# kessel/dune-pnp

Hardware: AMD Instinct MI355X
Metric: assembled DOFs/s + BiCGStab iters/s, 3-species PNP on pore.msh-refined (higher is better)
Workload: dtype f64; 1 GPU; config 3: stationary 3-ion PNP, test/pore_pnp/pore.msh refined k=4 x 1 mirrored copies; dofs=2214099, dofs_per_gpu=2214099, mesh_vertices=738033, triangles=1470464, parallelism=mesh partition (RCB) x1, preconditioner=ilu0, colors=4, sell_slots=5176768, blocks=5155025

## Files before the change

### dune-pnp_amd/csrc/assemble.hip

```cpp
#include <cstdlib>

#include <hip/hip_ext.h>

#include "element.h"
#include "kernels.h"

namespace pnp {

namespace {

template <int OP, int KC = 0>
__device__ __forceinline__ void store_block(double *__restrict__ vc, int lane, int s,
                                            const double *Kc) {
  constexpr int NK = OpTraits<OP>::NK;
  static_assert(!KC || OP == OP_PNP, "constant planes: the PNP operator only");
  constexpr int Q0 = KC ? 2 : 0;
#ifdef ASM_STORE_PLAIN
  store_vals<NK, Q0>(vc + size_t(s) * NK * kRows, lane, Kc);
#else
  store_vals_nt<NK, Q0>(vc + size_t(s) * NK * kRows, lane, Kc);
#endif
}

template <int NF>
__device__ __forceinline__ void residual_tail(const AsmArgs &a, int row, unsigned fl,
                                              const double (&R)[NF]) {
  double cv[NF];
#pragma unroll
  for (int f = 0; f < NF; f++) cv[f] = 0.0;
  if (fl & kRowFlagLoad) {
#pragma unroll
    for (int f = 0; f < NF; f++) cv[f] = a.cvec[size_t(row) * NF + f];
  }
#pragma unroll
  for (int f = 0; f < NF; f++) {
    const double rv = R[f] + cv[f];
    a.r[size_t(row) * NF + f] = ((fl >> f) & 1) ? 0.0 : rv;
  }
}

template <int OP, int JAC, int MINW, int FANR>
__global__ __launch_bounds__(256, MINW) void k_assemble(DevLayout L, AsmArgs a) {
  using T = OpTraits<OP>;
  constexpr int NF = T::NF, NK = T::NK;
  const int row = xcd_block(blockIdx.x, gridDim.x, L.xcd_remap) * blockDim.x + threadIdx.x;
  if (row >= L.n_owned) return;
  const int chunk = row / kRows, lane = row % kRows;
  const int off = L.chunk_off[chunk];
  const uint64_t meta = L.rowmeta[row];
  const int len = int(meta & 63);
  const bool closed = (meta >> 6) & 1;
  const unsigned brk = unsigned(meta >> 8);
  const int *__restrict__ cix = L.colidx + off + lane;
  double *__restrict__ vc = a.vals + size_t(off) * NK;

  const double2 pi2 = reinterpret_cast<const double2 *>(L.xy)[row];
  double ui[NF];
#pragma unroll
  for (int f = 0; f < NF; f++) ui[f] = a.x[size_t(row) * NF + f];
  double ai = 0, aq = 0;
  if constexpr (OP == OP_DIFF || OP == OP_DIFF_IE || OP == OP_POISSON) ai = a.aux0[row];
  if constexpr (OP == OP_POISSON) aq = a.aux1[row];
  if constexpr (OP == OP_PB) pb_fifth(ui[0], ai, aq);

  double R[NF], D[NK], P[NK], F[NK];
#pragma unroll
  for (int f = 0; f < NF; f++) R[f] = 0;
#pragma unroll
  for (int v = 0; v < NK; v++) D[v] = P[v] = F[v] = 0;

  auto next_slot = [&](int s) { return (s + 1 < len) ? s + 1 : (closed ? 1 : -1); };
  auto load_nb = [&](int j, double2 &p, double (&u)[NF], double &a0, double &a1) {
    p = reinterpret_cast<const double2 *>(L.xy)[j];
    load_nf<NF>(a.x, size_t(j), u);
    if constexpr (OP == OP_DIFF || OP == OP_DIFF_IE || OP == OP_POISSON) a0 = a.aux0[j];
    if constexpr (OP == OP_POISSON) a1 = a.aux1[j];
  };
  double2 pc, pn;
  double uc[NF], un[NF];
  double ac0 = 0, ac1 = 0, an0 = 0, an1 = 0;
  constexpr int NC = FANR > 0 ? FANR : 1;
  int cj[NC];
// ... 60 lines not shown
      for (int v = 0; v < NK; v++) P[v] = 0;
    }
    pc = pn;
#pragma unroll
    for (int f = 0; f < NF; f++) uc[f] = un[f];
    ac0 = an0;
    ac1 = an1;
    if (tn > 0) {
      pn = pp;
#pragma unroll
      for (int f = 0; f < NF; f++) un[f] = up[f];
      an0 = ap0;
      an1 = ap1;
    }
  }
  if constexpr (JAC) {
    if (closed) {
#pragma unroll
      for (int v = 0; v < NK; v++) F[v] += P[v];
      store_block<OP>(vc, lane, 1, F);
    }
    store_block<OP>(vc, lane, 0, D);
  }
  residual_tail<NF>(a, row, a.rowflag[row], R);
}

#ifndef ASM_SU
#define ASM_SU 4
#endif
template <int OP>
__host__ __device__ constexpr int asm_lds_rec() {
  return 2 + OpTraits<OP>::NF + (OP == OP_DIFF || OP == OP_DIFF_IE || OP == OP_POISSON) +
         (OP == OP_POISSON);
}
template <int OP>
constexpr int asm_kc() {
  return OP == OP_PNP;
}
constexpr int kPipeDw = 11;
template <class P>
__device__ __forceinline__ void lds_dma4(const P *src, uint32_t *dst_wave) {
  __builtin_amdgcn_global_load_lds(
      (const __attribute__((address_space(1))) void *)(src),
      (__attribute__((address_space(3))) void *)(dst_wave), 4, 0, 0);
}
__device__ __forceinline__ int const_ld(const int *p, int i) {
  return ((const __attribute__((address_space(4))) int *)(p))[i];
}
__device__ __forceinline__ int row_block_const(const DevLayout &L, int b, int nwg) {
  return L.blkmap ? const_ld(L.blkmap, xcd_block(b, nwg, 1)) : xcd_block(b, nwg, L.xcd_remap);
}
template <int OP, int JAC, int MINW, int FANR, int SPLIT = FANR, int STAGE = 0, int LDSG = 0,
          int KC = 0, int PIPE = 0>
__global__ __launch_bounds__(256, MINW) void k_assemble_ga(DevLayout L, AsmArgs a) {
  using T = OpTraits<OP>;
  constexpr int NF = T::NF, NK = T::NK, NS = FANR;
  constexpr bool AUX0 = OP == OP_DIFF || OP == OP_DIFF_IE || OP == OP_POISSON;
  constexpr bool AUX1 = OP == OP_POISSON;
  constexpr int RW = asm_lds_rec<OP>();
  static_assert(!PIPE || (JAC && FANR == 9 && !STAGE && !LDSG), "PIPE: the direct Jacobian walk");
  extern __shared__ double srec[];
  __shared__ uint32_t pfb[PIPE ? 4 * kPipeDw * kRows : 1];
  const int ntiles = (L.n_owned + 255) / 256, G = gridDim.x;
  const int wv = PIPE ? __builtin_amdgcn_readfirstlane(int(threadIdx.x) / kRows) : 0;
  const int ln = int(threadIdx.x) % kRows;
  uint32_t *const pw = pfb + (PIPE ? wv * kPipeDw * kRows : 0);
  int tile = blockIdx.x, b0 = -1, b1 = -1, b2 = -1, o0 = 0, o1 = 0, c1 = 0;
  auto tile_blk = [&](int t) { return t < ntiles ? row_block_const(L, t, ntiles) : -1; };
  auto wave_chunk = [&](int b) {
    return (b >= 0 && b * 256 + wv * kRows < L.n_owned) ? b * 4 + wv : -1;
  };
  auto prefetch = [&](int b, int off, int clen) {
    if (wave_chunk(b) < 0) return;
    const int r0 = b * 256 + wv * kRows;
    const int *cix = L.colidx + off + ln;
#pragma unroll
    for (int k = 1; k < NS; k++)
      lds_dma4(cix + (k < clen ? k : 0) * kRows, pw + (k - 1) * kRows);
    const uint32_t *m =
        reinterpret_cast<const uint32_t *>(L.rowmeta + min(r0 + ln, L.n_owned - 1));
    lds_dma4(m, pw + 8 * kRows);
    lds_dma4(m + 1, pw + 9 * kRows);
    lds_dma4(reinterpret_cast<const uint32_t *>(a.rowflag + r0) + (ln >> 2), pw + 10 * kRows);
  };
  if constexpr (PIPE) {
    if (tile >= ntiles) return;
    b0 = tile_blk(tile);
    b1 = tile_blk(tile + G);
    b2 = tile_blk(tile + 2 * G);
    int c0 = 0;
    if (wave_chunk(b0) >= 0) {
      o0 = const_ld(L.chunk_off, wave_chunk(b0));
      c0 = const_ld(L.chunk_len, wave_chunk(b0));
    }
    if (wave_chunk(b1) >= 0) {
      o1 = const_ld(L.chunk_off, wave_chunk(b1));
      c1 = const_ld(L.chunk_len, wave_chunk(b1));
    }
    prefetch(b0, o0, c0);
  }
  int o2 = 0, c2 = 0, b3 = -1;
  const auto advance = [&]() {
    tile += G;
    b0 = b1, o0 = o1;
    b1 = b2, o1 = o2, c1 = c2;
    b2 = b3;
    return b0 >= 0;
  };
  do {
    const int blk = PIPE ? b0 : row_block(L, blockIdx.x, gridDim.x);
    const int row0 = blk * blockDim.x + threadIdx.x;
    const bool live = row0 < L.n_owned;
    if (!PIPE && !LDSG && !live) return;
    const int row = live ? row0 : 0;
    const int chunk = row / kRows, lane = row % kRows;
    int cj[NS];
    uint64_t meta_pf = 0;
    unsigned fl_pf = 0;
    if constexpr (PIPE) {
      asm volatile("s_waitcnt vmcnt(0)" ::: "memory");
#pragma unroll
      for (int k = 1; k < NS; k++) cj[k] = int(pw[(k - 1) * kRows + ln]);
      meta_pf = uint64_t(pw[8 * kRows + ln]) | (uint64_t(pw[9 * kRows + ln]) << 32);
      fl_pf = (pw[10 * kRows + ln] >> (8 * (ln & 3))) & 0xffu;
      asm volatile("s_waitcnt lgkmcnt(0)" ::: "memory");
      prefetch(b1, o1, c1);
      o2 = c2 = 0;
      if (wave_chunk(b2) >= 0) {
        o2 = const_ld(L.chunk_off, wave_chunk(b2));
        c2 = const_ld(L.chunk_len, wave_chunk(b2));
      }
      b3 = tile_blk(tile + 3 * G);
      if (!live) continue;
    }
    const int off = PIPE ? o0 : L.chunk_off[chunk];
    const uint64_t meta = PIPE ? meta_pf : L.rowmeta[row];
    const int len = int(meta & 63);
    const bool closed = (meta >> 6) & 1;
    const unsigned brk = unsigned(meta >> 8);
    double *__restrict__ vc = a.vals + size_t(off) * NK;

    if constexpr (PIPE) {
    } else if constexpr (LDSG) {
      const uint16_t *__restrict__ lix = L.lidx + off + lane;
#pragma unroll
      for (int k = 1; k < NS; k++) {
        const int t = lix[(k < len ? k : 0) * kRows];
        cj[k] = k < len ? t : 0;
      }
    } else {
      const int *__restrict__ cix = L.colidx + off + lane;
#pragma unroll
      for (int k = 1; k < NS; k++) cj[k] = cix[(k < len ? k : 0) * kRows];
    }
    const double2 pi2 = reinterpret_cast<const double2 *>(L.xy)[row];
    double ui[NF];
    load_nf<NF>(a.x, size_t(row), ui);
    double ai = 0, aq = 0;
    if constexpr (AUX0) ai = a.aux0[row];
    if constexpr (AUX1) aq = a.aux1[row];
    if constexpr (OP == OP_PB) pb_fifth(ui[0], ai, aq);
    if constexpr (LDSG) {
      const int u0 = L.uptr[blk], cnt = L.uown[blk];
      constexpr int kSU = ASM_SU;
      int jj[kSU];
#pragma unroll
      for (int u = 0; u < kSU; u++) {
        const int k = int(threadIdx.x) + u * 256;
        jj[u] = k < cnt ? L.ulist[u0 + k] : -1;
      }
      double t[kSU][RW];
#pragma unroll
      for (int u = 0; u < kSU; u++)
        if (jj[u] >= 0) {
          const double2 p = reinterpret_cast<const double2 *>(L.xy)[jj[u]];
          t[u][0] = p.x;
          t[u][1] = p.y;
          double uu[NF];
          load_nf<NF>(a.x, size_t(jj[u]), uu);
#pragma unroll
// ... 100 lines not shown
#pragma unroll
              for (int v = 0; v < NK; v++) F[v] = P[v];
            } else {
              put(s, P);
            }
#pragma unroll
            for (int v = 0; v < NK; v++) P[v] = Ct[v];
          }
        } else if constexpr (JAC) {
          put(s, P);
#pragma unroll
          for (int v = 0; v < NK; v++) P[v] = 0;
        }
      }
    }
    if constexpr (JAC) {
      if (closed) {
#pragma unroll
        for (int v = 0; v < NK; v++) F[v] += P[v];
        store_block<OP, KC>(vc, lane, 1, F);
      }
      store_block<OP, KC>(vc, lane, 0, D);
    }
    residual_tail<NF>(a, row, PIPE ? fl_pf : unsigned(a.rowflag[row]), R);
  } while (PIPE && advance());
}

template <int OP>
__global__ __launch_bounds__(256) void k_mass_apply(DevLayout L, double tau, double pi, int cyl,
                                                    const double *__restrict__ xo,
                                                    double *__restrict__ cvec) {
  constexpr int NF = OpTraits<OP>::NF;
  const int row = blockIdx.x * blockDim.x + threadIdx.x;
  if (row >= L.n_owned) return;
  const int chunk = row / kRows, lane = row % kRows;
  const int off = L.chunk_off[chunk];
  const uint64_t meta = L.rowmeta[row];
  const int len = int(meta & 63);
  const bool closed = (meta >> 6) & 1;
  const int *cix = L.colidx + off + lane;
  const double2 pi2 = reinterpret_cast<const double2 *>(L.xy)[row];
  double acc = 0;
  for (int s = 1; s < len; ++s) {
    const int t = (s + 1 < len) ? s + 1 : (closed ? 1 : -1);
    if (t < 0 || ((meta >> (8 + s)) & 1)) continue;
    const int b = cix[s * kRows], c = cix[t * kRows];
    const double2 pb2 = reinterpret_cast<const double2 *>(L.xy)[b];
// ... 45 lines not shown
  double nx = ty / len, ny = -tx / len;
  if (nx * (po.x - pa.x) + ny * (po.y - pa.y) > 0) {
    nx = -nx;
    ny = -ny;
  }
  const double gp0 = factor * gf[0][0] * cp, gp1 = factor * gf[0][1] * cp;
  out[2 * size_t(k)] = (-factor * gf[1][0] + gp0) * nx + (-factor * gf[1][1] + gp1) * ny;
  const double r = cm / cp;
  out[2 * size_t(k) + 1] =
      (-factor * gf[2][0] - gp0 * r) * nx + (-factor * gf[2][1] - gp1 * r) * ny;
}

}

hipError_t launch_ion_flux(int ns, const int4 *seg, const double *xy, const double *x, int cyl,
                           double pi, double *out, hipStream_t s) {
  if (ns == 0) return hipSuccess;
  hipLaunchKernelGGL(k_ion_flux, dim3((ns + 255) / 256), dim3(256), 0, s, ns, seg, xy, x, cyl, pi,
                     out);
  return hipGetLastError();
}

constexpr bool kAsmPipeDefault = false;

template <int OP>
static int launch_pipe(const DevLayout &L, const AsmArgs &a, int cap, hipStream_t s, hipEvent_t t0,
                       hipEvent_t t1) {
  if constexpr (asm_kc<OP>()) {
    const auto kern = k_assemble_ga<OP, 1, 3, 9, 6, 0, 0, 1, 1>;
    static const int resident = [&] {
      int dev = 0, cus = 0, per_cu = 0;
      if (hipGetDevice(&dev) != hipSuccess ||
          hipDeviceGetAttribute(&cus, hipDeviceAttributeMultiprocessorCount, dev) != hipSuccess ||
          hipOccupancyMaxActiveBlocksPerMultiprocessor(&per_cu, kern, 256, 0) != hipSuccess)
        return 0;
      return per_cu * cus;
    }();
    const int ntiles = (L.n_owned + 255) / 256;
    int g = resident >= 8 ? resident / 8 * 8 : 8;
    if (g > ntiles) g = ntiles;
    if (cap > 0 && g > cap) g = cap;
    hipExtLaunchKernelGGL(kern, dim3(g), dim3(256), 0, s, t0, t1, 0, L, a);
    return 1;
  } else {
    return 0;
  }
// ... 18 lines not shown
  }();
  const int fanr = !fanr_ok ? 0 : (L.max_slots <= 9 ? 9 : (L.max_slots <= 12 ? 12 : 0));
  static const int lds_env = [] {
    const char *e = getenv("PNP_ASM_LDS");
    return e ? (atoi(e) == 1 ? 1 : 0) : -1;
  }();
  static const bool cold_hint = [] {
    const char *e = getenv("PNP_ASM_COLD_HINT");
    return !(e && e[0] == '0');
  }();
  const auto lds_walk = [&](int nk) {
    return lds_env == 1 ||
           (lds_env < 0 && (size_t(L.n_owned) * 7 * size_t(nk) * 8 > (size_t(512) << 20) ||
                            (cold_hint && a.cold)));
  };
  static const bool pipe_on = [] {
    const char *e = getenv("PNP_ASM_PIPE");
    return e ? atoi(e) != 0 : kAsmPipeDefault;
  }();
  static const int pipe_cap = [] {
    const char *e = getenv("PNP_ASM_PIPE_GRID");
    return (e && atoi(e) >= 1) ? atoi(e) : 0;
  }();
  int piped = 0;
#define PNP_ASM_CASE(OPK)                                                          \
  case OPK:                                                                        \
    if (!fanr && a.jac)                                                            \
      hipExtLaunchKernelGGL((k_assemble<OPK, 1, 3, 0>), grid, block, 0, s, t0, t1, 0, L, a);     \
    else if (!fanr)                                                                \
      hipExtLaunchKernelGGL((k_assemble<OPK, 0, 4, 0>), grid, block, 0, s, t0, t1, 0, L, a);     \
    else if (!a.jac && fanr == 9 && ga && lds_env == 1 && L.uown &&                 \
             size_t(L.unmax) * asm_lds_rec<OPK>() * 8 <= 53 * 1024)                    \
      hipExtLaunchKernelGGL((k_assemble_ga<OPK, 0, 3, 9, 9, 0, 1>), grid, block,         \
                         size_t(L.unmax) * asm_lds_rec<OPK>() * 8, s, t0, t1, 0, L, a);             \
    else if (!a.jac && fanr == 9 && ga)                                            \
      hipExtLaunchKernelGGL((k_assemble_ga<OPK, 0, 3, 9>), grid, block, 0, s, t0, t1, 0, L, a);  \
    else if (!a.jac)                                                               \
      hipExtLaunchKernelGGL((k_assemble<OPK, 0, 4, 12>), grid, block, 0, s, t0, t1, 0, L, a);    \
    else if (ga == 1 && fanr == 9)                                                 \
      hipExtLaunchKernelGGL((k_assemble_ga<OPK, 1, 3, 9>), grid, block, 0, s, t0, t1, 0, L, a);  \
    else if (ga == 2 && fanr == 9)                                                 \
      hipExtLaunchKernelGGL((k_assemble_ga<OPK, 1, 2, 9>), grid, block, 0, s, t0, t1, 0, L, a);  \
    else if (ga == 3 && fanr == 9)                                                 \
      hipExtLaunchKernelGGL((k_assemble_ga<OPK, 1, 3, 9, 5>), grid, block, 0, s, t0, t1, 0, L, a); \
    else if (ga == 4 && fanr == 9 && asm_kc<OPK>() && a.kconst &&                   \
             lds_walk(OpTraits<OPK>::NK) && L.uown &&                               \
             size_t(L.unmax) * asm_lds_rec<OPK>() * 8 <= 53 * 1024)                    \
      hipExtLaunchKernelGGL((k_assemble_ga<OPK, 1, 3, 9, 6, 0, 1, asm_kc<OPK>()>), grid,  \
                         block, size_t(L.unmax) * asm_lds_rec<OPK>() * 8, s, t0, t1, 0, L, a); \
    else if (ga == 4 && fanr == 9 && asm_kc<OPK>() && a.kconst && pipe_on)         \
      piped = launch_pipe<OPK>(L, a, pipe_cap, s, t0, t1);                         \
    else if (ga == 4 && fanr == 9 && asm_kc<OPK>() && a.kconst)                    \
      hipExtLaunchKernelGGL((k_assemble_ga<OPK, 1, 3, 9, 6, 0, 0, asm_kc<OPK>()>), grid,  \
                         block, 0, s, t0, t1, 0, L, a);                             \
    else if (ga == 4 && fanr == 9 && lds_walk(OpTraits<OPK>::NK) && L.uown &&       \
             size_t(L.unmax) * asm_lds_rec<OPK>() * 8 <= 53 * 1024)                    \
      hipExtLaunchKernelGGL((k_assemble_ga<OPK, 1, 3, 9, 6, 0, 1>), grid, block,         \
                         size_t(L.unmax) * asm_lds_rec<OPK>() * 8, s, t0, t1, 0, L, a);             \
    else if (ga == 4 && fanr == 9)                                                 \
      hipExtLaunchKernelGGL((k_assemble_ga<OPK, 1, 3, 9, 6>), grid, block, 0, s, t0, t1, 0, L, a); \
    else if (ga == 5 && fanr == 9)                                                 \
      hipExtLaunchKernelGGL((k_assemble_ga<OPK, 1, 3, 9, 3>), grid, block, 0, s, t0, t1, 0, L, a); \
    else if (ga == 6 && fanr == 9)                                                 \
      hipExtLaunchKernelGGL((k_assemble_ga<OPK, 1, 3, 9, 6, 1>), grid, block, 0, s, t0, t1, 0, L, a); \
    else if (fanr == 12)                                                           \
      hipExtLaunchKernelGGL((k_assemble<OPK, 1, 3, 12>), grid, block, 0, s, t0, t1, 0, L, a);    \
    else if (waves == 3)                                                           \
      hipExtLaunchKernelGGL((k_assemble<OPK, 1, 3, 9>), grid, block, 0, s, t0, t1, 0, L, a);     \
    else                                                                           \
      hipExtLaunchKernelGGL((k_assemble<OPK, 1, 4, 9>), grid, block, 0, s, t0, t1, 0, L, a);     \
    break;
  switch (a.kind) {
    PNP_ASM_CASE(OP_PNP)
    PNP_ASM_CASE(OP_PNP_IE)
    PNP_ASM_CASE(OP_PB)
    PNP_ASM_CASE(OP_DIFF)
    PNP_ASM_CASE(OP_DIFF_IE)
    PNP_ASM_CASE(OP_POISSON)
  default:
    return hipErrorInvalidValue;
  }
#undef PNP_ASM_CASE
  if (pipelined) *pipelined = piped;
  return hipGetLastError();
}

hipError_t launch_mass_apply(const DevLayout &L, int kind, double tau, double pi, int cylindrical,
                             const double *x_old, double *cvec, hipStream_t s) {
  if (L.n_owned == 0) return hipSuccess;
  dim3 grid((L.n_owned + 255) / 256), block(256);
  if (kind == OP_PNP_IE)
    hipLaunchKernelGGL(k_mass_apply<OP_PNP_IE>, grid, block, 0, s, L, tau, pi, cylindrical, x_old,
                       cvec);
  else if (kind == OP_DIFF_IE)
    hipLaunchKernelGGL(k_mass_apply<OP_DIFF_IE>, grid, block, 0, s, L, tau, pi, cylindrical,
                       x_old, cvec);
  else
    return hipErrorInvalidValue;
  return hipGetLastError();
}

}
```

### dune-pnp_amd/csrc/ctx.cc

```cpp
#include <hip/hip_runtime.h>
#include <rccl/rccl.h>
#include <rocsolver/rocsolver.h>

#include <algorithm>
#include <queue>
#include <random>
#include <chrono>
#include <condition_variable>
#include <map>
#include <unordered_map>
#include <mutex>
#include <cmath>
#include <cstdio>
#include <cstdlib>
#include <cstring>
#include <memory>
#include <string>
#include <vector>

#include "../../include/pnp_capi.h"
#include "amg.h"
#include "gmres_small.h"
#include "idr_small.h"
#include "kernels.h"
// ... 107 lines not shown
      d_usrc;
  DBuf<double> lvals, uvals, tsgs;
  int split_of = 0;
  int ilu_f32 = [] {
    const char *e = std::getenv("PNP_ILU_F32");
    const int v = e ? std::atoi(e) : 2;
    return (v >= 0 && v <= 3) ? v : 2;
  }();
  int ilu_eff() const { return (ilu_f32 >= 2 && nf == 1) ? 1 : ilu_f32; }
  int ilu_fac() const { return ilu_eff() == 3 ? 2 : ilu_eff(); }
  int f32_now() const { return split_of == 2 ? ilu_fac() : 0; }
  DBuf<float> ilu_y32buf;
  float *ilu_y32() const {
    return (split_of == 2 && ilu_eff() == 3 && !ilu_flow_opt) ? ilu_y32buf.p : nullptr;
  }
  int ilu_fused = 1;
  int amg_fallback = 0;
  int ilu_retry = 1;
  int twored_opt = [] {
    const char *ev = std::getenv("PNP_BICG_TWORED");
    return ev ? (std::atoi(ev) != 0 ? 1 : 0) : -1;
  }();
  DBuf<int> d_blkmap;
  DBuf<int> d_rowoff, d_rowcol;
  DBuf<int> d_blk_int, d_blk_bnd;
  int n_blk_int = 0, n_blk_bnd = 0;
  bool split_spmv = false;
  pnp::DevLayout sub_layout(bool interior) const {
    pnp::DevLayout d = dl;
    d.blkmap = interior ? d_blk_int.p : d_blk_bnd.p;
    const int n = interior ? n_blk_int : n_blk_bnd;
    d.blkcount = n > 0 ? n : -1;
    return d;
  }
  hipStream_t cstream = nullptr;
  hipEvent_t ev_ready = nullptr, ev_halo = nullptr;
  DBuf<double> scrub;
  bool fd_built = false, fd_mode = false;
  int fd_opt = 0;
  int fd_ne = 0;
  DBuf<int> fd_etri, fd_cdata;
  DBuf<long long> fd_rptr;
  DBuf<double> fd_jel;
  int csr_pat = -1, csr_nf = 0;
  long long csr_nnz = 0;
  DBuf<int> csr_rowptr, csr_col, csr_src;
// ... 3183 lines not shown
    if ((rc = up(c->d_rowoff, ro, "rowoff")) || (rc = up(c->d_rowcol, rcol, "rowcol"))) {
      g_err = c->err;
      return rc;
    }
  }
  {
    const char *e = getenv("PNP_BLKMAP");
    if (!(e && atoi(e) == 0) && L.n_owned > 0) {
      int nblk = (L.n_owned + 255) / 256;
      std::vector<double> key(nblk);
      for (int b = 0; b < nblk; b++) {
        int r = 256 * b, cc = L.rowcolor[r];
        double lo = L.color_ptr[cc], hi = L.color_ptr[cc + 1];
        key[b] = (r - lo) / std::max(1.0, hi - lo);
      }
      std::vector<int> order(nblk);
      for (int b = 0; b < nblk; b++) order[b] = b;
      std::stable_sort(order.begin(), order.end(), [&](int a, int b) { return key[a] < key[b]; });
      if ((rc = up(c->d_blkmap, order, "blkmap"))) {
        g_err = c->err;
        return rc;
      }
      c->dl.blkmap = c->d_blkmap.p;
    }
  }
  {
    const pnp::Mesh &mg = c->mesh;
    auto ekey = [](int a, int b) {
      if (a > b) std::swap(a, b);
      return (long long)a << 32 | (unsigned)b;
    };
    std::unordered_map<long long, int> opp;
    opp.reserve(size_t(mg.nb) * 2);
    for (int b = 0; b < mg.nb; b++) opp[ekey(mg.bseg[2 * b], mg.bseg[2 * b + 1])] = -1;
    for (int e = 0; e < mg.nt; e++)
      for (int k = 0; k < 3; k++) {
        auto it = opp.find(ekey(mg.tri[3 * e + k], mg.tri[3 * e + (k + 1) % 3]));
        if (it != opp.end() && it->second < 0) it->second = mg.tri[3 * e + (k + 2) % 3];
      }
    std::vector<int4> segs;
    for (int b = 0; b < mg.nb; b++) {
      const int a = mg.bseg[2 * b], cc = mg.bseg[2 * b + 1], lo = L.g2l[std::min(a, cc)];
      if (lo < 0 || lo >= L.n_owned) continue;
      const int o = opp[ekey(a, cc)];
      const int la = L.g2l[a], lc = L.g2l[cc], lop = o >= 0 ? L.g2l[o] : -1;
      if (la < 0 || lc < 0 || lop < 0) {
// ... 7 lines not shown
      g_err = c->err;
      return rc;
    }
  }
  c->dl.lchunk_len = c->d_lchunk_len.p;
  c->dl.lchunk_off = c->d_lchunk_off.p;
  c->dl.lcolidx = c->d_lcolidx.p;
  c->dl.uchunk_len = c->d_uchunk_len.p;
  c->dl.uchunk_off = c->d_uchunk_off.p;
  c->dl.ucolidx = c->d_ucolidx.p;
  if ((rc = up(c->d_chunk_len, L.chunk_len, "chunk_len")) ||
      (rc = up(c->d_chunk_off, L.chunk_off, "chunk_off")) ||
      (rc = up(c->d_colidx, L.colidx, "colidx")) || (rc = up(c->d_rowmeta, L.rowmeta, "rowmeta")) ||
      (rc = up(c->d_xy, xy, "xy")) || (rc = up(c->d_l2g, L.l2g, "l2g")) ||
      (rc = up(c->d_send_idx, L.send_idx, "send_idx")) ||
      (rc = up(c->d_color_idx, L.color_idx, "color_idx")) ||
      (rc = up(c->d_rowcolor, L.rowcolor, "rowcolor"))) {
    g_err = c->err;
    return rc;
  }
  {
    const char *e = getenv("PNP_XCD_REMAP");
    c->dl.xcd_remap = (e && atoi(e) == 1) ? 1 : 0;
  }
  c->dl.n_owned = L.n_owned;
  c->dl.n_local = nloc;
  c->dl.nchunks = L.nchunks;
  c->dl.max_slots = L.chunk_len.empty() ? 0 : *std::max_element(L.chunk_len.begin(), L.chunk_len.end());
  c->dl.ncolors = int(L.color_ptr.size()) - 1;
  c->dl.chunk_len = c->d_chunk_len.p;
  c->dl.chunk_off = c->d_chunk_off.p;
  c->dl.colidx = c->d_colidx.p;
  c->dl.rowmeta = c->d_rowmeta.p;
  if (const char *ev = getenv("PNP_SPMV_LDS"); !(ev && atoi(ev) == 0)) {
    const int nblk = (L.n_owned + 255) / 256;
    std::vector<int> uptr(nblk + 1, 0), ulist;
    std::vector<uint16_t> lidx(size_t(L.nslots), 0);
    std::vector<int> cols, uown(nblk, 0);
    int umax = 0, unmax = 0;
    bool fits = true;
    const bool own_last = [] {
      const char *e = getenv("PNP_LIST_OWN_LAST");
      return !(e && e[0] == '0');
    }();
    for (int b = 0; b < nblk && fits; b++) {
      cols.clear();
// ... 855 lines not shown
  if (!c) return PNP_E_ARG;
  if (replacements) *replacements = c->idr_replacements;
  return PNP_OK;
}

extern "C" int pnp_idr_shadow(pnp_ctx *c, int32_t j, double *p) {
  if (!c || !p) return PNP_E_ARG;
  if (!c->idr_P.p || c->idr_P_s != c->idr_s || c->idr_P_nf != c->nf)
    return c->fail(PNP_E_STATE, "no IDR solve yet with the current PNP_OPT_IDR_S and operator");
  if (j < 0 || j >= c->idr_s) return c->fail(PNP_E_ARG, "shadow column out of range");
  hipSetDevice(c->device);
  return c->download_ext(c->idr_P.p + size_t(j) * size_t(c->idr_ld(false)), c->nf, p);
}

extern "C" int pnp_asm_row_flags(pnp_ctx *c, uint8_t *flags) {
  if (!c || !flags) return PNP_E_ARG;
  if (c->kind < 0) return c->fail(PNP_E_STATE, "no operator set (pnp_set_operator)");
  if (c->degree > 1) return c->fail(PNP_E_STATE, "row flags: P1 contexts only");
  std::memset(flags, 0xff, size_t(c->mesh.nv));
  for (int i = 0; i < c->L.n_owned; i++) flags[c->L.l2g[i]] = c->hrowflag[i];
  return PNP_OK;
}

extern "C" int pnp_asm_info(pnp_ctx *c, int64_t *full, int64_t *reused, int64_t *pipelined) {
  if (!c) return PNP_E_ARG;
  if (full) *full = c->asm_full;
  if (reused) *reused = c->asm_reused;
  if (pipelined) *pipelined = c->asm_piped;
  return PNP_OK;
}

extern "C" int pnp_amg_configure(pnp_ctx *c, const pnp_amg_opts *o) {
  if (!c || !o) return PNP_E_ARG;
  if (o->smoother != PNP_PREC_SSOR && o->smoother != PNP_PREC_ILU0 &&
      o->smoother != PNP_PREC_JACOBI && o->smoother != PNP_PREC_SSOR_NATURAL)
    return c->fail(PNP_E_ARG, "AMG smoother must be SSOR, SSOR_NATURAL, ILU0 or JACOBI");
  if (o->coarse_target < 1 || o->coarse_target > pnp::kAmgMaxCoarse || o->max_levels < 2 ||
      o->max_levels > pnp::kAmgMaxLevels || !(o->omega > 0 && o->omega <= 2) ||
      o->coarse_sweeps < 1 || o->coarse_sweeps > 8 || o->level0_presmooth < -1 ||
      o->level0_presmooth > 1)
    return c->fail(PNP_E_ARG, "AMG options out of range");
  const bool rebuild = o->coarse_target != c->amg_opts.coarse_target ||
                       o->max_levels != c->amg_opts.max_levels;
  c->amg_opts = *o;
  if (rebuild) c->amg_built = false;
  c->amg_valid = false;
// ... 685 lines not shown
```

### dune-pnp_amd/csrc/kernels.h

```cpp
#pragma once

#include <hip/hip_runtime.h>

#include <cstdint>

namespace pnp {

constexpr int kRows = 64;

__device__ __forceinline__ int xcd_block(int b, int nwg, int on = 1) {
  if (!on) return b;
  const int q = nwg / 8, r = nwg % 8, xcd = b % 8;
  return (xcd < r ? xcd * (q + 1) : r * (q + 1) + (xcd - r) * q) + b / 8;
}

typedef double double2_a8 __attribute__((ext_vector_type(2), aligned(8)));
template <int NF>
__device__ __forceinline__ void load_nf(const double *__restrict__ x, size_t j, double (&o)[NF]) {
  const double *b = x + size_t(NF) * j;
  int f = 0;
#pragma unroll
  for (; f + 1 < NF; f += 2) {
    const double2_a8 a = *reinterpret_cast<const double2_a8 *>(b + f);
    o[f] = a.x;
    o[f + 1] = a.y;
  }
  if (f < NF) o[f] = b[f];
}
template <int NF>
__device__ __forceinline__ void store_nf(double *__restrict__ x, size_t j, const double (&v)[NF]) {
  double *b = x + size_t(NF) * j;
  int f = 0;
#pragma unroll
// ... 130 lines not shown
template <int NF, int PAT>
__host__ __device__ __forceinline__ void mask_rows(double *B, unsigned dm, bool diag) {
#pragma unroll
  for (int f = 0; f < NF; f++)
#pragma unroll
    for (int g = 0; g < NF; g++) {
      const int v = pat_index(PAT, f, g);
      if (v >= 0 && ((dm >> f) & 1)) B[v] = (diag && f == g) ? 1.0 : 0.0;
    }
}

struct DevLayout {
  int n_owned = 0, n_local = 0, nchunks = 0, ncolors = 0;
  int max_slots = 0;
  int xcd_remap = 0;
  const int *chunk_len = nullptr;
  const int *chunk_off = nullptr;
  const int *colidx = nullptr;
  const uint64_t *rowmeta = nullptr;
  const double *xy = nullptr;
  const int *color_idx = nullptr;
  const uint8_t *rowcolor = nullptr;
  const int *blkmap = nullptr;
  int blkcount = 0;
  const int *lchunk_len = nullptr, *lchunk_off = nullptr, *lcolidx = nullptr;
  const int *uchunk_len = nullptr, *uchunk_off = nullptr, *ucolidx = nullptr;
  const uint8_t *dmask = nullptr;
  const int *uptr = nullptr, *ulist = nullptr;
  const uint16_t *lidx = nullptr;
  int umax = 0;
  const int *uown = nullptr;
  int unmax = 0;
  const int *lsx_ptr = nullptr, *lsx_list = nullptr, *usx_ptr = nullptr, *usx_list = nullptr;
  const uint8_t *lperm = nullptr, *uperm = nullptr, *lpinv = nullptr, *upinv = nullptr;
  const uint8_t *llen = nullptr, *ulen = nullptr, *ldl = nullptr;
  const uint16_t *lsx_idx = nullptr, *usx_idx = nullptr;
  int sx_max = 0;
};

template <int NF>
__device__ __forceinline__ unsigned row_mask(const DevLayout &L, int row) {
  unsigned dm = 0;
#pragma unroll
  for (int f = 0; f < NF; f++) dm |= unsigned(L.dmask[size_t(row) * NF + f] != 0) << f;
  return dm;
}

constexpr unsigned kRowFlagMask = 7, kRowFlagLoad = 8;

struct AsmArgs {
  int kind;
  int jac;
  double l_b, c0, tau, pi, dt, z;
  int cylindrical;
  const double *x;
  const double *aux0;
  const double *aux1;
  const double *cvec;
  const uint8_t *dmask;
  const uint8_t *rowflag;
  double *r;
// ... 234 lines not shown
```

### dune-pnp_amd/python/pnp_amd/__init__.py

```python
from __future__ import annotations

import ctypes as C
import os
from dataclasses import dataclass

import numpy as np

HERE = os.path.dirname(os.path.abspath(__file__))
PKG_ROOT = os.path.dirname(os.path.dirname(HERE))
REPO_ROOT = os.path.dirname(PKG_ROOT)
LIB_PATH = os.environ.get("PNP_AMD_LIB") or os.path.join(PKG_ROOT, "libpnp_amd.so")
HEADER = os.path.join(REPO_ROOT, "include", "pnp_capi.h")

OK, E_ARG, E_HIP, E_RCCL, E_BREAKDOWN, E_NOT_CONVERGED, E_IO, E_MESH, E_STATE = \
    0, -1, -2, -3, -4, -5, -6, -7, -8
OP_PNP, OP_PNP_IMPLICIT_EULER, OP_PB, OP_DIFF, OP_DIFF_IMPLICIT_EULER, OP_POISSON = range(6)
PREC_NONE, PREC_SSOR, PREC_ILU0, PREC_JACOBI, PREC_AMG, PREC_SSOR_NATURAL = range(6)
METHOD_BICGSTAB, METHOD_CG, METHOD_GMRES, METHOD_FGMRES, METHOD_IDR = 0, 1, 2, 3, 4
(OPT_ILU_F32, OPT_ILU_FUSED_FACTOR, OPT_JAC_FD, OPT_BICG_TWORED, OPT_AMG_FALLBACK,
 OPT_GRAPH, OPT_SEQ_ORDER, OPT_ILU_FLOW, OPT_NAT_FLOW, OPT_ILU_RETRY,
 OPT_GMRES_RESTART, OPT_MATRIX_FREE, OPT_ASM_REUSE_CONST, OPT_IDR_S) = (1, 2, 3, 4, 5, 6, 7, 8,
                                                                        9, 10, 11, 12, 13, 14)
ASM_PIPE_ENV, ASM_PIPE_GRID_ENV = "PNP_ASM_PIPE", "PNP_ASM_PIPE_GRID"
ROW_FLAG_LOAD = 8
DEVICE_PTRS, JAC_FD = 1, 2
CREATE_ABSORB_THIN_COLOR = 1
PREC_BY_NAME = {"none": PREC_NONE, "nonprec": PREC_NONE, "ssor": PREC_SSOR, "ilu0": PREC_ILU0,
                "jacobi": PREC_JACOBI, "amg": PREC_AMG, "ssor_natural": PREC_SSOR_NATURAL}
MAX_SURFACES = 64


class PnpError(RuntimeError):
    def __init__(self, code, msg):
        super().__init__(f"pnp error {code}: {msg}")
        self.code = code


class _Mesh(C.Structure):
    _fields_ = [("nv", C.c_int32), ("coords", C.c_void_p), ("nt", C.c_int32),
                ("tri", C.c_void_p), ("nbseg", C.c_int32), ("bseg", C.c_void_p),
                ("bseg_group", C.c_void_p)]


class _Surface(C.Structure):
    _fields_ = [("coulomb_btype", C.c_int32), ("coulomb_flux", C.c_double),
                ("coulomb_potential", C.c_double), ("plus_btype", C.c_int32),
                ("plus_flux", C.c_double), ("plus_concentration", C.c_double),
# ... 700 lines not shown
    def asm_row_flags(self):
        out = np.zeros(self.mesh.nv, dtype=np.uint8)
        self._ck(lib().pnp_asm_row_flags(self.h, out.ctypes.data_as(C.c_void_p)))
        return out

    def probe_slot_stores(self, tile_elems=256, reps=20):
        o = _StoreProbe()
        self._ck(lib().pnp_probe_slot_stores(self.h, int(tile_elems), int(reps), C.byref(o)))
        return {k: getattr(o, k) for k, _ in _StoreProbe._fields_}

    def cache_scrub(self, nbytes=1 << 30):
        self._ck(lib().pnp_cache_scrub(self.h, C.c_int64(int(nbytes))))

    def timers(self, enable=None, reset=False):
        if enable is not None:
            self._ck(lib().pnp_timers_enable(self.h, int(bool(enable))))
        if reset:
            self._ck(lib().pnp_timers_reset(self.h))
        t = _Timers()
        self._ck(lib().pnp_timers_get(self.h, C.byref(t)))
        return {k: getattr(t, k) for k, _ in _Timers._fields_}


def header_symbols():
    import re
    txt = open(HEADER).read()
    return sorted(set(re.findall(r"^\s*(?:int|void|const char \*)\s*(pnp_\w+)\s*\(", txt, re.M)))


def header_constants():
    import re
    txt = open(HEADER).read()
    return {k: int(v) for k, v in re.findall(r"^\s*(PNP_\w+)\s*=\s*(-?\d+)\s*,?\s*$", txt, re.M)}
```

### include/pnp_capi.h

```cpp
#ifndef PNP_CAPI_H
#define PNP_CAPI_H

#include <stdint.h>

#ifdef __cplusplus
extern "C" {
#endif

#define PNP_CAPI_VERSION 1

enum {
  PNP_OK = 0,
  PNP_E_ARG = -1,
  PNP_E_HIP = -2,
  PNP_E_RCCL = -3,
  PNP_E_BREAKDOWN = -4,
  PNP_E_NOT_CONVERGED = -5,
  PNP_E_IO = -6,
  PNP_E_MESH = -7,
  PNP_E_STATE = -8
};

typedef struct pnp_ctx pnp_ctx;

// ... 181 lines not shown
  double omega;
} pnp_amg_stats;
int pnp_amg_info(pnp_ctx *ctx, pnp_amg_stats *stats);
int pnp_amg_aggregates(pnp_ctx *ctx, int32_t level, int32_t *agg);

enum {
  PNP_OPT_ILU_F32 = 1,
  PNP_OPT_ILU_FUSED_FACTOR = 2,
  PNP_OPT_JAC_FD = 3,
  PNP_OPT_BICG_TWORED = 4,
  PNP_OPT_AMG_FALLBACK = 5,
  PNP_OPT_GRAPH = 6,
  PNP_OPT_SEQ_ORDER = 7,
  PNP_OPT_ILU_FLOW = 8,
  PNP_OPT_NAT_FLOW = 9,
  PNP_OPT_ILU_RETRY = 10,
  PNP_OPT_GMRES_RESTART = 11,
  PNP_OPT_MATRIX_FREE = 12,
  PNP_OPT_ASM_REUSE_CONST = 13,
  PNP_OPT_IDR_S = 14
};
int pnp_set_option(pnp_ctx *ctx, int32_t option, int64_t value);
int pnp_asm_info(pnp_ctx *ctx, int64_t *full, int64_t *reused, int64_t *pipelined);
#define PNP_ROW_FLAG_LOAD 8
int pnp_asm_row_flags(pnp_ctx *ctx, uint8_t *flags);
int pnp_matfree_info(pnp_ctx *ctx, int64_t *applies, int64_t *value_assemblies);
int pnp_idr_info(pnp_ctx *ctx, int64_t *replacements);
int pnp_idr_shadow(pnp_ctx *ctx, int32_t j, double *p);

enum {
  PNP_CREATE_ABSORB_THIN_COLOR = 1
};
int pnp_set_create_option(int32_t option, int64_t value);
int pnp_get_create_option(int32_t option, int64_t *value);
int pnp_get_option(pnp_ctx *ctx, int32_t option, int64_t *value);

int pnp_linear_solve(pnp_ctx *ctx, const double *rhs, double *z, const pnp_solve_opts *opts,
                     pnp_solve_result *res);
int pnp_linear_solve_ex(pnp_ctx *ctx, const double *rhs, double *z, const pnp_solve_opts *opts,
                        pnp_solve_result *res, int32_t flags);

int pnp_solve_history(pnp_ctx *ctx, double *defects, int32_t cap, int32_t *n);

typedef struct {
  double reduction, abs_limit, min_linear_reduction;
  int32_t maxit, line_search_maxit;
// ... 80 lines not shown
```

Measured before the change: 55.29 billion assembled DOFs/s.

## Launch direct assembly walks as one-wave workgroups driven by a precomputed unit table

Builds a host-side table of per-wave assembly units holding the chunk index, offset and length, ordered by XCD and block map, and uploads it to the device. The non-pipelined direct assembly kernels now read this table through scalar constant loads instead of computing the block index and loading chunk_off per wave. They are launched by default as 64-thread workgroups, one wave per unit, in place of 256-thread blocks. The rowflag load is also moved earlier, next to the other row loads, to hide its latency. This trades an extra table and a different scheduling granularity for fewer dependent address loads at kernel start and finer wave dispatch.

Result: no change. 55.77 billion assembled DOFs/s, median of 6 (+0.9%).

```diff
diff --git a/dune-pnp_amd/csrc/assemble.hip b/dune-pnp_amd/csrc/assemble.hip
--- a/dune-pnp_amd/csrc/assemble.hip
+++ b/dune-pnp_amd/csrc/assemble.hip
@@ -37,6 +37,21 @@
     const double rv = R[f] + cv[f];
     a.r[size_t(row) * NF + f] = ((fl >> f) & 1) ? 0.0 : rv;
   }
+}
+
+__device__ __forceinline__ unsigned head_flag(const AsmArgs &a, int row) {
+#ifdef ASM_FLAG_TAIL
+  return 0;
+#else
+  return a.rowflag[row];
+#endif
+}
+__device__ __forceinline__ unsigned tail_flag(const AsmArgs &a, int row, unsigned fl) {
+#ifdef ASM_FLAG_TAIL
+  return a.rowflag[row];
+#else
+  return fl;
+#endif
 }
 
 template <int OP, int JAC, int MINW, int FANR>
@@ -58,6 +73,7 @@
   double ui[NF];
 #pragma unroll
   for (int f = 0; f < NF; f++) ui[f] = a.x[size_t(row) * NF + f];
+  const unsigned fl = head_flag(a, row);
   double ai = 0, aq = 0;
   if constexpr (OP == OP_DIFF || OP == OP_DIFF_IE || OP == OP_POISSON) ai = a.aux0[row];
   if constexpr (OP == OP_POISSON) aq = a.aux1[row];
@@ -164,7 +180,7 @@
     }
     store_block<OP>(vc, lane, 0, D);
   }
-  residual_tail<NF>(a, row, a.rowflag[row], R);
+  residual_tail<NF>(a, row, tail_flag(a, row, fl), R);
 }
 
 #ifndef ASM_SU
@@ -189,22 +205,37 @@
 __device__ __forceinline__ int const_ld(const int *p, int i) {
   return ((const __attribute__((address_space(4))) int *)(p))[i];
 }
+__device__ __forceinline__ int4 unit_ld(const int4 *p, int i) {
+  typedef int i4v __attribute__((ext_vector_type(4)));
+  const i4v e = ((const __attribute__((address_space(4))) i4v *)(p))[i];
+  return make_int4(e.x, e.y, e.z, e.w);
+}
+#ifdef ASM_HEAD_CHAIN
+constexpr bool kAsmUnits = false;
+#else
+constexpr bool kAsmUnits = true;
+#endif
 __device__ __forceinline__ int row_block_const(const DevLayout &L, int b, int nwg) {
   return L.blkmap ? const_ld(L.blkmap, xcd_block(b, nwg, 1)) : xcd_block(b, nwg, L.xcd_remap);
 }
 template <int OP, int JAC, int MINW, int FANR, int SPLIT = FANR, int STAGE = 0, int LDSG = 0,
-          int KC = 0, int PIPE = 0>
-__global__ __launch_bounds__(256, MINW) void k_assemble_ga(DevLayout L, AsmArgs a) {
+          int KC = 0, int PIPE = 0, int WG = 256>
+__global__ __launch_bounds__(WG, MINW) void k_assemble_ga(DevLayout L, AsmArgs a) {
   using T = OpTraits<OP>;
   constexpr int NF = T::NF, NK = T::NK, NS = FANR;
   constexpr bool AUX0 = OP == OP_DIFF || OP == OP_DIFF_IE || OP == OP_POISSON;
   constexpr bool AUX1 = OP == OP_POISSON;
   constexpr int RW = asm_lds_rec<OP>();
   static_assert(!PIPE || (JAC && FANR == 9 && !STAGE && !LDSG), "PIPE: the direct Jacobian walk");
+  static_assert(WG == 256 || (WG == kRows && kAsmUnits && !PIPE && !STAGE && !LDSG),
+                "one-wave workgroups: the walks without LDS, by the unit table");
+  constexpr bool UNITS = kAsmUnits && !PIPE;
   extern __shared__ double srec[];
   __shared__ uint32_t pfb[PIPE ? 4 * kPipeDw * kRows : 1];
   const int ntiles = (L.n_owned + 255) / 256, G = gridDim.x;
-  const int wv = PIPE ? __builtin_amdgcn_readfirstlane(int(threadIdx.x) / kRows) : 0;
+  const int wv = (PIPE || (UNITS && WG == 256))
+                     ? __builtin_amdgcn_readfirstlane(int(threadIdx.x) / kRows)
+                     : 0;
   const int ln = int(threadIdx.x) % kRows;
   uint32_t *const pw = pfb + (PIPE ? wv * kPipeDw * kRows : 0);
   int tile = blockIdx.x, b0 = -1, b1 = -1, b2 = -1, o0 = 0, o1 = 0, c1 = 0;
@@ -250,9 +281,24 @@
     return b0 >= 0;
   };
   do {
-    const int blk = PIPE ? b0 : row_block(L, blockIdx.x, gridDim.x);
-    const int row0 = blk * blockDim.x + threadIdx.x;
-    const bool live = row0 < L.n_owned;
+    int blk = 0, row0 = 0, off_u = 0, clen_u = 0;
+    bool live;
+    if constexpr (UNITS) {
+#ifndef ASM_KARG_LATE
+      asm volatile("" ::"s"(L.n_owned), "s"(L.colidx), "s"(L.rowmeta), "s"(L.xy), "s"(a.x),
+                   "s"(a.rowflag));
+#endif
+      const int b = blockIdx.x, u0 = (4 * (b / 8)) * 8 + b % 8;
+      const int4 e = unit_ld(L.units, WG == kRows ? b : u0 + 8 * wv);
+      if constexpr (LDSG) blk = unit_ld(L.units, u0).x / 4;
+      off_u = e.y, clen_u = e.z;
+      row0 = e.x * kRows + ln;
+      live = e.x >= 0 && row0 < L.n_owned;
+    } else {
+      blk = PIPE ? b0 : row_block(L, blockIdx.x, gridDim.x);
+      row0 = blk * blockDim.x + threadIdx.x;
+      live = row0 < L.n_owned;
+    }
     if (!PIPE && !LDSG && !live) return;
     const int row = live ? row0 : 0;
     const int chunk = row / kRows, lane = row % kRows;
@@ -275,7 +321,7 @@
       b3 = tile_blk(tile + 3 * G);
       if (!live) continue;
     }
-    const int off = PIPE ? o0 : L.chunk_off[chunk];
+    const int off = PIPE ? o0 : (UNITS ? off_u : L.chunk_off[chunk]);
     const uint64_t meta = PIPE ? meta_pf : L.rowmeta[row];
     const int len = int(meta & 63);
     const bool closed = (meta >> 6) & 1;
@@ -287,17 +333,18 @@
       const uint16_t *__restrict__ lix = L.lidx + off + lane;
 #pragma unroll
       for (int k = 1; k < NS; k++) {
-        const int t = lix[(k < len ? k : 0) * kRows];
+        const int t = lix[(k < (UNITS ? clen_u : len) ? k : 0) * kRows];
         cj[k] = k < len ? t : 0;
       }
     } else {
       const int *__restrict__ cix = L.colidx + off + lane;
 #pragma unroll
-      for (int k = 1; k < NS; k++) cj[k] = cix[(k < len ? k : 0) * kRows];
+      for (int k = 1; k < NS; k++) cj[k] = cix[(k < (UNITS ? clen_u : len) ? k : 0) * kRows];
     }
     const double2 pi2 = reinterpret_cast<const double2 *>(L.xy)[row];
     double ui[NF];
     load_nf<NF>(a.x, size_t(row), ui);
+    const unsigned fl_hd = PIPE ? 0u : head_flag(a, row);
     double ai = 0, aq = 0;
     if constexpr (AUX0) ai = a.aux0[row];
     if constexpr (AUX1) aq = a.aux1[row];
@@ -444,7 +491,7 @@
       }
       store_block<OP, KC>(vc, lane, 0, D);
     }
-    residual_tail<NF>(a, row, PIPE ? fl_pf : unsigned(a.rowflag[row]), R);
+    residual_tail<NF>(a, row, PIPE ? fl_pf : tail_flag(a, row, fl_hd), R);
   } while (PIPE && advance());
 }
 
@@ -536,6 +583,8 @@
 }
 
 constexpr bool kAsmPipeDefault = false;
+constexpr int kAsmWgDefault = kRows;
+constexpr int kAsmWg1 = kAsmUnits ? kRows : 256;
 
 template <int OP>
 static int launch_pipe(const DevLayout &L, const AsmArgs &a, int cap, hipStream_t s, hipEvent_t t0,
@@ -600,7 +649,26 @@
     const char *e = getenv("PNP_ASM_PIPE_GRID");
     return (e && atoi(e) >= 1) ? atoi(e) : 0;
   }();
+  static const int wg = [] {
+    const char *e = getenv("PNP_ASM_WG");
+    const int v = e ? atoi(e) : 0;
+    return (v == 64 || v == 256) && kAsmUnits ? v : (kAsmUnits ? kAsmWgDefault : 256);
+  }();
+  if (kAsmUnits && !L.units) return hipErrorInvalidValue;
+  const dim3 grid1(unsigned(asm_unit_count(L.n_owned))), block1(kRows);
   int piped = 0;
+#define PNP_ASM_DIRECT(OPK, JAC, SPLIT, KC)                                                     \
+  do {                                                                                          \
+    if constexpr (kAsmUnits) {                                                                  \
+      if (wg == kRows) {                                                                        \
+        hipExtLaunchKernelGGL((k_assemble_ga<OPK, JAC, 3, 9, SPLIT, 0, 0, KC, 0, kAsmWg1>),     \
+                              grid1, block1, 0, s, t0, t1, 0, L, a);                            \
+        break;                                                                                  \
+      }                                                                                         \
+    }                                                                                           \
+    hipExtLaunchKernelGGL((k_assemble_ga<OPK, JAC, 3, 9, SPLIT, 0, 0, KC>), grid, block, 0, s,  \
+                          t0, t1, 0, L, a);                                                     \
+  } while (0)
 #define PNP_ASM_CASE(OPK)                                                          \
   case OPK:                                                                        \
     if (!fanr && a.jac)                                                            \
@@ -612,7 +680,7 @@
       hipExtLaunchKernelGGL((k_assemble_ga<OPK, 0, 3, 9, 9, 0, 1>), grid, block,         \
                          size_t(L.unmax) * asm_lds_rec<OPK>() * 8, s, t0, t1, 0, L, a);             \
     else if (!a.jac && fanr == 9 && ga)                                            \
-      hipExtLaunchKernelGGL((k_assemble_ga<OPK, 0, 3, 9>), grid, block, 0, s, t0, t1, 0, L, a);  \
+      PNP_ASM_DIRECT(OPK, 0, 9, 0);                                                \
     else if (!a.jac)                                                               \
       hipExtLaunchKernelGGL((k_assemble<OPK, 0, 4, 12>), grid, block, 0, s, t0, t1, 0, L, a);    \
     else if (ga == 1 && fanr == 9)                                                 \
@@ -629,14 +697,13 @@
     else if (ga == 4 && fanr == 9 && asm_kc<OPK>() && a.kconst && pipe_on)         \
       piped = launch_pipe<OPK>(L, a, pipe_cap, s, t0, t1);                         \
     else if (ga == 4 && fanr == 9 && asm_kc<OPK>() && a.kconst)                    \
-      hipExtLaunchKernelGGL((k_assemble_ga<OPK, 1, 3, 9, 6, 0, 0, asm_kc<OPK>()>), grid,  \
-                         block, 0, s, t0, t1, 0, L, a);                             \
+      PNP_ASM_DIRECT(OPK, 1, 6, asm_kc<OPK>());                                    \
     else if (ga == 4 && fanr == 9 && lds_walk(OpTraits<OPK>::NK) && L.uown &&       \
              size_t(L.unmax) * asm_lds_rec<OPK>() * 8 <= 53 * 1024)                    \
       hipExtLaunchKernelGGL((k_assemble_ga<OPK, 1, 3, 9, 6, 0, 1>), grid, block,         \
                          size_t(L.unmax) * asm_lds_rec<OPK>() * 8, s, t0, t1, 0, L, a);             \
     else if (ga == 4 && fanr == 9)                                                 \
-      hipExtLaunchKernelGGL((k_assemble_ga<OPK, 1, 3, 9, 6>), grid, block, 0, s, t0, t1, 0, L, a); \
+      PNP_ASM_DIRECT(OPK, 1, 6, 0);                                                \
     else if (ga == 5 && fanr == 9)                                                 \
       hipExtLaunchKernelGGL((k_assemble_ga<OPK, 1, 3, 9, 3>), grid, block, 0, s, t0, t1, 0, L, a); \
     else if (ga == 6 && fanr == 9)                                                 \
@@ -659,6 +726,7 @@
     return hipErrorInvalidValue;
   }
 #undef PNP_ASM_CASE
+#undef PNP_ASM_DIRECT
   if (pipelined) *pipelined = piped;
   return hipGetLastError();
 }
diff --git a/dune-pnp_amd/csrc/ctx.cc b/dune-pnp_amd/csrc/ctx.cc
--- a/dune-pnp_amd/csrc/ctx.cc
+++ b/dune-pnp_amd/csrc/ctx.cc
@@ -153,6 +153,8 @@
     return ev ? (std::atoi(ev) != 0 ? 1 : 0) : -1;
   }();
   DBuf<int> d_blkmap;
+  std::vector<int> h_blkmap;
+  DBuf<int> d_units;
   DBuf<int> d_rowoff, d_rowcol;
   DBuf<int> d_blk_int, d_blk_bnd;
   int n_blk_int = 0, n_blk_bnd = 0;
@@ -3382,6 +3384,7 @@
         return rc;
       }
       c->dl.blkmap = c->d_blkmap.p;
+      c->h_blkmap = order;
     }
   }
   {
@@ -3435,6 +3438,17 @@
   {
     const char *e = getenv("PNP_XCD_REMAP");
     c->dl.xcd_remap = (e && atoi(e) == 1) ? 1 : 0;
+  }
+  if (L.n_owned > 0) {
+    std::vector<int> units(4 * pnp::asm_unit_count(L.n_owned));
+    pnp::asm_unit_table(L.n_owned, L.chunk_off.data(), L.chunk_len.data(),
+                        c->h_blkmap.empty() ? nullptr : c->h_blkmap.data(), c->dl.xcd_remap,
+                        units.data());
+    if ((rc = up(c->d_units, units, "assembly units"))) {
+      g_err = c->err;
+      return rc;
+    }
+    c->dl.units = reinterpret_cast<const int4 *>(c->d_units.p);
   }
   c->dl.n_owned = L.n_owned;
   c->dl.n_local = nloc;
@@ -4336,6 +4350,17 @@
   return PNP_OK;
 }
 
+extern "C" int pnp_asm_unit_table(int32_t n_owned, const int32_t *chunk_off,
+                                  const int32_t *chunk_len, const int32_t *blkmap,
+                                  int32_t xcd_remap, int32_t *table, int64_t capacity) {
+  if (n_owned < 0 || (n_owned > 0 && (!chunk_off || !chunk_len))) return -1;
+  const int n = int(pnp::asm_unit_count(n_owned));
+  if (!table) return n;
+  if (capacity < n) return -1;
+  pnp::asm_unit_table(n_owned, chunk_off, chunk_len, blkmap, xcd_remap ? 1 : 0, table);
+  return n;
+}
+
 extern "C" int pnp_asm_info(pnp_ctx *c, int64_t *full, int64_t *reused, int64_t *pipelined) {
   if (!c) return PNP_E_ARG;
   if (full) *full = c->asm_full;
diff --git a/dune-pnp_amd/csrc/kernels.h b/dune-pnp_amd/csrc/kernels.h
--- a/dune-pnp_amd/csrc/kernels.h
+++ b/dune-pnp_amd/csrc/kernels.h
@@ -8,7 +8,7 @@
 
 constexpr int kRows = 64;
 
-__device__ __forceinline__ int xcd_block(int b, int nwg, int on = 1) {
+__host__ __device__ __forceinline__ int xcd_block(int b, int nwg, int on = 1) {
   if (!on) return b;
   const int q = nwg / 8, r = nwg % 8, xcd = b % 8;
   return (xcd < r ? xcd * (q + 1) : r * (q + 1) + (xcd - r) * q) + b / 8;
@@ -185,6 +185,7 @@
   const int *color_idx = nullptr;
   const uint8_t *rowcolor = nullptr;
   const int *blkmap = nullptr;
+  const int4 *units = nullptr;
   int blkcount = 0;
   const int *lchunk_len = nullptr, *lchunk_off = nullptr, *lcolidx = nullptr;
   const int *uchunk_len = nullptr, *uchunk_off = nullptr, *ucolidx = nullptr;
@@ -200,6 +201,31 @@
   const uint16_t *lsx_idx = nullptr, *usx_idx = nullptr;
   int sx_max = 0;
 };
+
+inline size_t asm_unit_count(int n_owned) {
+  const int ntiles = (n_owned + 255) / 256;
+  return size_t(8) * 4 * size_t((ntiles + 7) / 8);
+}
+inline void asm_unit_table(int n_owned, const int *chunk_off, const int *chunk_len,
+                           const int *blkmap, int xcd_remap, int *out) {
+  const int ntiles = (n_owned + 255) / 256, nchunks = (n_owned + kRows - 1) / kRows;
+  const int P = 4 * ((ntiles + 7) / 8);
+  for (int p = 0; p < P; p++)
+    for (int x = 0; x < 8; x++) {
+      const int b = 8 * (p / 4) + x;
+      int chunk = -1;
+      if (b < ntiles) {
+        const int blk = blkmap ? blkmap[xcd_block(b, ntiles, 1)] : xcd_block(b, ntiles, xcd_remap);
+        chunk = 4 * blk + p % 4;
+        if (chunk >= nchunks) chunk = -1;
+      }
+      int *e = out + 4 * (size_t(p) * 8 + x);
+      e[0] = chunk;
+      e[1] = chunk >= 0 ? chunk_off[chunk] : 0;
+      e[2] = chunk >= 0 ? chunk_len[chunk] : 0;
+      e[3] = 0;
+    }
+}
 
 template <int NF>
 __device__ __forceinline__ unsigned row_mask(const DevLayout &L, int row) {
diff --git a/dune-pnp_amd/python/pnp_amd/__init__.py b/dune-pnp_amd/python/pnp_amd/__init__.py
--- a/dune-pnp_amd/python/pnp_amd/__init__.py
+++ b/dune-pnp_amd/python/pnp_amd/__init__.py
@@ -23,6 +23,7 @@
                                                                         9, 10, 11, 12, 13, 14)
 ASM_PIPE_ENV, ASM_PIPE_GRID_ENV = "PNP_ASM_PIPE", "PNP_ASM_PIPE_GRID"
 ROW_FLAG_LOAD = 8
+ASM_WG_ENV = "PNP_ASM_WG"
 DEVICE_PTRS, JAC_FD = 1, 2
 CREATE_ABSORB_THIN_COLOR = 1
 PREC_BY_NAME = {"none": PREC_NONE, "nonprec": PREC_NONE, "ssor": PREC_SSOR, "ilu0": PREC_ILU0,
@@ -769,6 +770,26 @@
         return {k: getattr(t, k) for k, _ in _Timers._fields_}
 
 
+def asm_unit_table(n_owned, chunk_off, chunk_len, blkmap=None, xcd_remap=0):
+    co = np.ascontiguousarray(chunk_off, dtype=np.int32)
+    cl = np.ascontiguousarray(chunk_len, dtype=np.int32)
+    bm = None if blkmap is None else np.ascontiguousarray(blkmap, dtype=np.int32)
+    ip = C.POINTER(C.c_int32)
+    f = lib().pnp_asm_unit_table
+    f.restype = C.c_int
+    f.argtypes = [C.c_int32, ip, ip, ip, C.c_int32, ip, C.c_int64]
+    n = f(int(n_owned), co.ctypes.data_as(ip), cl.ctypes.data_as(ip),
+          None if bm is None else bm.ctypes.data_as(ip), int(xcd_remap), None, 0)
+    if n < 0:
+        raise PnpError(E_ARG, "pnp_asm_unit_table: bad argument")
+    out = np.zeros((n, 4), dtype=np.int32)
+    if f(int(n_owned), co.ctypes.data_as(ip), cl.ctypes.data_as(ip),
+         None if bm is None else bm.ctypes.data_as(ip), int(xcd_remap),
+         out.ctypes.data_as(ip), n) != n:
+        raise PnpError(E_ARG, "pnp_asm_unit_table: bad argument")
+    return out
+
+
 def header_symbols():
     import re
     txt = open(HEADER).read()
diff --git a/include/pnp_capi.h b/include/pnp_capi.h
--- a/include/pnp_capi.h
+++ b/include/pnp_capi.h
@@ -227,6 +227,8 @@
 };
 int pnp_set_option(pnp_ctx *ctx, int32_t option, int64_t value);
 int pnp_asm_info(pnp_ctx *ctx, int64_t *full, int64_t *reused, int64_t *pipelined);
+int pnp_asm_unit_table(int32_t n_owned, const int32_t *chunk_off, const int32_t *chunk_len,
+                       const int32_t *blkmap, int32_t xcd_remap, int32_t *table, int64_t capacity);
 #define PNP_ROW_FLAG_LOAD 8
 int pnp_asm_row_flags(pnp_ctx *ctx, uint8_t *flags);
 int pnp_matfree_info(pnp_ctx *ctx, int64_t *applies, int64_t *value_assemblies);
```
